# matteociccozzi/LayoutDiT

Hardware: AMD Instinct MI355X
Metric: images/sec ViT-B/16 224px bs=64 fwd (higher is better)
Workload: dtype f32; 1 GPU; ViT-base/16 224x224 bs=64 f32 forward, taps [4, 6, 8, 12] (BASELINE.json configs[1]); images_per_gpu=64, global_batch=64, parallelism=dp1: batch-sharded replicas, no data-path collective, weights=synthetic seed 0, images=synthetic doc-like pages, seed 1234, rank0_placement=128 CPUs: NUMA node 0 of GPU 0000:72:00.0

## Files before the change

include/ldit.h:

```cpp
#ifndef LDIT_H
#define LDIT_H

#include <stddef.h>
#include <stdint.h>

#ifdef __cplusplus
extern "C" {
#endif

#define LDIT_ABI_VERSION 6
#define LDIT_MAX_TAPS 8

enum ldit_status {
    LDIT_OK = 0,
    LDIT_EINVAL = -1,
    LDIT_EWORKSPACE = -2,
    LDIT_EHIP = -3,
    LDIT_EUNSUPPORTED = -4
};

enum ldit_dtype {
    LDIT_F32 = 0,
    LDIT_BF16 = 1,
    LDIT_FP8 = 3,
// ... 41 lines not shown
    const void *wq, *bq;
    const void *wk;
    const void *wv, *bv;
    const void *wo, *bo;
    const void *lam1;
    const void *ln2_w, *ln2_b;
    const void *w1, *b1;
    const void *w2, *b2;
    const void *lam2;
} ldit_layer_weights;

typedef struct ldit_weights {
    const void *patch_w;
    const void *patch_b;
    const void *cls;
    const void *pos;
    const ldit_layer_weights *layer;
} ldit_weights;

int ldit_abi_version(void);
const char *ldit_last_error(void);
int ldit_debug_reload_env(void);


size_t ldit_packed_bytes(const ldit_cfg *cfg);

int ldit_pack_weights(const ldit_cfg *cfg, const ldit_weights *w, void *packed, size_t packed_bytes, ldit_stream stream);

int ldit_set_fp8_act_scales(const ldit_cfg *cfg, void *packed, size_t packed_bytes, const float *act_scales,
                            ldit_stream stream);

size_t ldit_workspace_bytes(const ldit_cfg *cfg, int32_t batch);

int ldit_vit_forward(const ldit_cfg *cfg, const void *packed, const void *x, int32_t batch, void *const *tap_out,
                     void *workspace, size_t workspace_bytes, ldit_stream stream);

int ldit_vit_forward_images(const ldit_cfg *cfg, const void *packed, const void *const *images, const int32_t *heights,
                            const int32_t *widths, int32_t half_in, float mean, float std, int32_t batch, void *const *tap_out,
                            void *workspace, size_t workspace_bytes, ldit_stream stream);

enum ldit_kernel_family {
    LDIT_K_GEMM = 0,
    LDIT_K_ATTENTION = 1,
    LDIT_K_LAYERNORM = 2,
    LDIT_K_OTHER = 3,
    LDIT_K_COUNT = 4
};
int ldit_vit_forward_timed(const ldit_cfg *cfg, const void *packed, const void *x, int32_t batch, void *const *tap_out,
                           void *workspace, size_t workspace_bytes, ldit_stream stream, double *ms, int64_t *launches);


int ldit_linear_f32(const void *X, int64_t lda, const void *W, const void *bias, void *Y, int64_t ldy, int64_t M,
                    int64_t N, int64_t K, int32_t epilogue, const void *lam, const void *R, void *Y2,
                    ldit_stream stream);

int ldit_layernorm_f32(const void *X, const void *gamma, const void *beta, void *Y, int64_t rows, int64_t C, float eps,
                       ldit_stream stream);

int ldit_attention_f32(const void *Q, const void *K, const void *V, void *O, int64_t B, int64_t N, int64_t H,
                       int64_t D, int64_t ldq, int64_t ldk, int64_t ldv, int64_t ldo, float scale, ldit_stream stream);

int ldit_embed_f32(const void *x, const void *patch_w, const void *patch_b, const void *cls, const void *pos, void *out,
                   int64_t B, int64_t in_ch, int64_t img_h, int64_t img_w, int64_t p, int64_t C, ldit_stream stream);

int ldit_tap_to_map_f32(const void *tap, void *out, int64_t B, int64_t Gh, int64_t Gw, int64_t C, float scale,
                        ldit_stream stream);
// ... 200 lines not shown
```

layoutdit_amd/_lib.py:

```python
from __future__ import annotations

import ctypes as C
import os

_HERE = os.path.dirname(os.path.abspath(__file__))
LIB_PATH = os.environ.get("LDIT_LIB_PATH") or os.path.join(_HERE, "libldit_hip.so")

LDIT_ABI_VERSION = 6
LDIT_MAX_TAPS = 8
DTYPE_F32, DTYPE_BF16, DTYPE_FP8, DTYPE_F32X3, DTYPE_F32X6, DTYPE_MXFP8 = 0, 1, 3, 4, 5, 6
FP8_A_COUNT = 4
LDIT_OK, LDIT_EINVAL, LDIT_EWORKSPACE, LDIT_EHIP, LDIT_EUNSUPPORTED = 0, -1, -2, -3, -4
EPI_BIAS, EPI_BIAS_GELU, EPI_SCALE_RESID, EPI_F32, EPI_GELU_BWD = 0, 1, 2, 4, 5
K_GEMM, K_ATTENTION, K_LAYERNORM, K_OTHER, K_COUNT = 0, 1, 2, 3, 4
KERNEL_FAMILIES = ("gemm", "attention", "layernorm", "other")


class LditCfg(C.Structure):
    _fields_ = [("hidden", C.c_int32), ("layers", C.c_int32), ("heads", C.c_int32), ("mlp", C.c_int32),
                ("patch", C.c_int32), ("in_ch", C.c_int32), ("img_h", C.c_int32), ("img_w", C.c_int32),
                ("n_taps", C.c_int32), ("taps", C.c_int32 * LDIT_MAX_TAPS), ("ln_eps", C.c_float),
                ("dtype", C.c_int32), ("flags", C.c_int32)]


# ... 2 lines not shown


class LditLayerWeights(C.Structure):
    _fields_ = [(n, C.c_void_p) for n in LAYER_FIELDS]


class LditWeights(C.Structure):
    _fields_ = [("patch_w", C.c_void_p), ("patch_b", C.c_void_p), ("cls", C.c_void_p), ("pos", C.c_void_p),
                ("layer", C.POINTER(LditLayerWeights))]


class LditOptSegment(C.Structure):
    _fields_ = [("p", C.c_void_p), ("g", C.c_void_p), ("m", C.c_void_p), ("v", C.c_void_p), ("n", C.c_int64),
                ("bf16_mirror", C.c_void_p)]


class LditOptState(C.Structure):
    _fields_ = [("found_inf", C.c_int32), ("skip", C.c_int32), ("step", C.c_int32), ("growth_tracker", C.c_int32),
                ("skipped_steps", C.c_int32), ("scale", C.c_float), ("inv_scale_used", C.c_float), ("lr", C.c_float),
                ("bc1", C.c_float), ("bc2_sqrt", C.c_float)]


OPT_STATE_FIELDS = tuple(n for n, _ in LditOptState._fields_)
OPT_MAX_SEGMENTS = 64

_vp, _i64, _i32, _f32, _sz = C.c_void_p, C.c_int64, C.c_int32, C.c_float, C.c_size_t
SIGNATURES = {
    "ldit_abi_version": (C.c_int, []),
    "ldit_last_error": (C.c_char_p, []),
    "ldit_debug_reload_env": (C.c_int, []),
    "ldit_packed_bytes": (_sz, [C.POINTER(LditCfg)]),
    "ldit_pack_weights": (C.c_int, [C.POINTER(LditCfg), C.POINTER(LditWeights), _vp, _sz, _vp]),
    "ldit_workspace_bytes": (_sz, [C.POINTER(LditCfg), _i32]),
    "ldit_vit_forward": (C.c_int, [C.POINTER(LditCfg), _vp, _vp, _i32, C.POINTER(_vp), _vp, _sz, _vp]),
    "ldit_vit_forward_images": (C.c_int, [C.POINTER(LditCfg), _vp, C.POINTER(_vp), C.POINTER(_i32), C.POINTER(_i32), _i32, _f32, _f32, _i32,
                                          C.POINTER(_vp), _vp, _sz, _vp]),
    "ldit_vit_forward_timed": (C.c_int, [C.POINTER(LditCfg), _vp, _vp, _i32, C.POINTER(_vp), _vp, _sz, _vp,
                                         C.POINTER(C.c_double), C.POINTER(C.c_int64)]),
    "ldit_linear_f32": (C.c_int, [_vp, _i64, _vp, _vp, _vp, _i64, _i64, _i64, _i64, _i32, _vp, _vp, _vp, _vp]),
    "ldit_layernorm_f32": (C.c_int, [_vp, _vp, _vp, _vp, _i64, _i64, _f32, _vp]),
    "ldit_attention_f32": (C.c_int, [_vp, _vp, _vp, _vp, _i64, _i64, _i64, _i64, _i64, _i64, _i64, _i64, _f32, _vp]),
    "ldit_embed_f32": (C.c_int, [_vp, _vp, _vp, _vp, _vp, _vp, _i64, _i64, _i64, _i64, _i64, _i64, _vp]),
    "ldit_attention_planes": (C.c_int, [_vp, _vp, _vp, _vp, _i64, _i64, _i64, _i64, _i64, _i64, _i64, _i32, _vp]),
    "ldit_split_f32_planes": (C.c_int, [_vp, _i64, _vp, _i64, _i64, _i32, _vp]),
    "ldit_layernorm_f32_planes": (C.c_int, [_vp, _vp, _vp, _vp, _i64, _i64, C.c_float, _i32, _vp]),
    "ldit_linear_planes": (C.c_int, [_vp, _i64, _vp, _vp, _vp, _i64, _i64, _i64, _i64, _i32, _vp, _vp, _vp, _i32, _vp]),
    "ldit_embed_bf16": (C.c_int, [_vp, _vp, _vp, _vp, _vp, _vp, _vp, _i64, _i64, _i64, _i64, _i64, _i64, _vp]),
    "ldit_embed_bf16_images": (C.c_int, [C.POINTER(_vp), C.POINTER(_i32), C.POINTER(_i32), _i32, _f32, _f32, _vp, _vp, _vp, _vp, _vp, _vp,
                                         _i64, _i64, _i64, _i64, _i64, _i64, _vp]),
    "ldit_tap_to_map_f32": (C.c_int, [_vp, _vp, _i64, _i64, _i64, _i64, _f32, _vp]),
    "ldit_tap_to_map_bwd_f32": (C.c_int, [_vp, _vp, _i64, _i64, _i64, _i64, _f32, _vp]),
    "ldit_linear_bf16": (C.c_int, [_vp, _i64, _vp, _vp, _vp, _i64, _i64, _i64, _i64, _i32, _vp, _vp, _vp, _vp]),
    "ldit_attention_bf16": (C.c_int, [_vp, _vp, _vp, _vp, _i64, _i64, _i64, _i64, _i64, _i64, _i64, _i64, _f32, _vp]),
    "ldit_cast_f32_bf16": (C.c_int, [_vp, _vp, _i64, _vp]),
    "ldit_linear_fp8": (C.c_int, [_vp, _i64, _vp, _vp, _vp, _i64, _i64, _i64, _i64, _i32, _vp, _vp, _vp, _f32, _f32, _vp, _vp]),
    "ldit_quant_rows_f32_fp8": (C.c_int, [_vp, _vp, _vp, _i64, _i64, _vp]),
    "ldit_set_fp8_act_scales": (C.c_int, [C.POINTER(LditCfg), _vp, C.c_size_t, C.POINTER(C.c_float), _vp]),
    "ldit_quant_f32_fp8": (C.c_int, [_vp, _vp, _i64, _f32, _vp]),
    "ldit_quant_mx_f32_fp8": (C.c_int, [_vp, _i64, _vp, _vp, _i64, _i64, _vp]),
    "ldit_linear_mxfp8": (C.c_int, [_vp, _i64, _vp, _vp, _vp, _vp, _vp, _i64, _vp, _i64, _i64, _i64, _i32, _vp, _vp, _vp, _vp]),
    "ldit_layernorm_mxfp8": (C.c_int, [_vp, _vp, _vp, _vp, _vp, _i64, _i64, _f32, _vp]),
    "ldit_amax_f32": (C.c_int, [_vp, _i64, _vp, _vp]),
    "ldit_preprocess_f32": (C.c_int, [C.POINTER(_vp), C.POINTER(_i32), C.POINTER(_i32), _i32, _i32, _f32, _f32, _i32, _i32,
                                      _vp, _vp]),
    "ldit_preprocess_f16": (C.c_int, [C.POINTER(_vp), C.POINTER(_i32), C.POINTER(_i32), _i32, _i32, _f32, _f32, _i32, _i32,
                                      _vp, _vp]),
# ... 108 lines not shown
```

layoutdit_amd/csrc/api.hip:

```cpp
#include "api_internal.h"

namespace ldit {

char *err_buf()
{
    static thread_local char buf[512] = {0};
    return buf;
}

int fail(int code, const char *fmt, ...)
{
    va_list ap;
    va_start(ap, fmt);
    vsnprintf(err_buf(), 512, fmt, ap);
    va_end(ap);
    return code;
}

int ensure_dynamic_lds(const void *kern, int bytes, std::atomic<unsigned long long> &done)
{
    int dev = 0;
    LDIT_HIP_CHECK(hipGetDevice(&dev));
    const unsigned long long bit = dev >= 0 && dev < 64 ? 1ull << dev : 0ull;
    if (bit && (done.load(std::memory_order_relaxed) & bit)) return LDIT_OK;
    LDIT_HIP_CHECK(hipFuncSetAttribute(kern, hipFuncAttributeMaxDynamicSharedMemorySize, bytes));
    if (bit) done.fetch_or(bit, std::memory_order_relaxed);
    return LDIT_OK;
}

int compute_units()
{
    static std::atomic<int> cached[64];
    int dev = 0;
// ... 4 lines not shown
        if (c > 0) return c;
    }
    int n = 0;
    if (hipDeviceGetAttribute(&n, hipDeviceAttributeMultiprocessorCount, dev) != hipSuccess || n <= 0) n = 256;
    if (slot) cached[dev].store(n, std::memory_order_relaxed);
    return n;
}

namespace {
DiagSwitches read_switches()
{
    DiagSwitches d;
    auto digit = [](const char *name, int lo, int hi) {
        const char *e = getenv(name);
        return (e && e[0] >= '0' + lo && e[0] <= '0' + hi && e[1] == 0) ? e[0] - '0' : -1;
    };
    auto is = [](const char *name, char c) { const char *e = getenv(name); return e && e[0] == c; };
    d.gemm_tile = digit("LDIT_GEMM_TILE", 0, 7);
    if (const char *e = getenv("LDIT_GEMM_THIN_TILES")) d.thin_tiles = atol(e);
    d.panel_r16_vec = is("LDIT_PANEL_R16", 'v');
    d.panel_persist = is("LDIT_GEMM_PERSIST", '1');
    d.bf16_tile = digit("LDIT_GEMM_BF16_TILE", 2, 7);
    d.bf16_tile_env = getenv("LDIT_GEMM_BF16_TILE") != nullptr;
    d.bf16_tr_tile = digit("LDIT_GEMM_BF16_TR_TILE", 0, 9);
    d.bf16_tail_launch = is("LDIT_GEMM_BF16_TAIL_LAUNCH", '1');
    d.fp8_tile = digit("LDIT_GEMM_FP8_TILE", 0, 6);
    d.fp8_k16 = is("LDIT_GEMM_FP8_K16", '1');
    d.fp8_noskinny = is("LDIT_GEMM_FP8_NOSKINNY", '1');
    d.direct_epi = is("LDIT_GEMM_DIRECT_EPILOGUE", '1');
    d.attn_bf16_kt4 = is("LDIT_ATTN_BF16_KT", '4');
    d.seg_order = digit("LDIT_GEMM_SEG_ORDER", 0, 1);
    if (const char *e = getenv("LDIT_PLANES_TAIL_WAVES")) d.planes_tail_waves = atol(e);
    d.attn_bf16_nw = digit("LDIT_ATTN_BF16_NW", 4, 8);
    return d;
}
DiagSwitches &switches()
{
    static DiagSwitches d = read_switches();
    return d;
}
}

const DiagSwitches &diag() { return switches(); }
void reload_diag() { switches() = read_switches(); }

int embed(const Geo &g, const float *x, const float *pw, const float *pb, const float *cls, const float *pos, float *out,
          int batch, int img_h, int img_w, hipStream_t stream, Probe &probe)
{
    GemmArgs a{};
    a.A = x; a.W = pw; a.Y = out; a.Y2 = nullptr; a.bias = pb; a.pos = pos;
    a.M = batch * g.P; a.N = g.C; a.K = g.Kp;
    a.lda = g.in_ch * img_h * img_w;
    a.ldy = g.C;
    a.img_h = img_h; a.img_w = img_w; a.gw = g.gw; a.patches = g.P; a.patch = g.p; a.tokens = g.T;
    LDIT_RUN(probe, LDIT_K_GEMM, launch_gemm(a, EPI_EMBED, A_PATCH, stream));
    LDIT_RUN(probe, LDIT_K_OTHER, launch_cls_rows(cls, pos, out, batch, g.T, g.C, stream));
    return LDIT_OK;
}

int embed_bf16(const Geo &g, const float *x, const ImgSrc *imgs, int planes, void *patches, const void *w16, const float *pb,
               const float *cls, const float *pos, float *out, int batch, int img_h, int img_w, hipStream_t stream, Probe &probe)
{
    if (imgs)
        LDIT_RUN(probe, LDIT_K_OTHER, launch_patches_rows_images(imgs->images, imgs->half_in, imgs->heights, imgs->widths, batch, g.in_ch,
                                                                imgs->mean, imgs->std, img_h, img_w, g.p, patches, stream, planes));
    else
// ... 39 lines not shown
        }
        case LDIT_FP8:
            return launch_gemm_fp8(A.p, A.ld, W, bias, Y.p, Y.ld, M, N, K, epi, lam, R, Y2, ab_scale, out_inv_scale,
                                   static_cast<const float *>(A.s), static_cast<const float *>(Ws), static_cast<const float *>(Y.s), stream);
        case LDIT_MXFP8:
            if (b.train && epi != EPI_BIAS)
                return launch_gemm_mxfp8_train(A.p, A.ld, A.s, W, Ws, bias, Y.p, Y.ld, Y.s, M, N, K, epi, lam, R, Y2, t.Ypre, t.rowscale, t.Yd, stream);
            return launch_gemm_mxfp8(A.p, A.ld, A.s, W, Ws, bias, Y.p, Y.ld, Y.s, M, N, K, epi, lam, R, Y2, stream);
        default: return fail(LDIT_EUNSUPPORTED, "linear: no kernel for dtype %d", b.dtype);
    }
}

int attention(Build b, const void *Q, const void *K, const void *V, int ldq, int ldk, int ldv, const Operand &O, int B, int N, int H, int D,
              float scale, hipStream_t stream, float *lse, void *Ob, void *Od, int plane_in)
{
    switch (b.dtype) {
        case LDIT_F32:
            return launch_attention(static_cast<const float *>(Q), static_cast<const float *>(K), static_cast<const float *>(V),
                                    static_cast<float *>(O.p), B, N, H, D, ldq, ldk, ldv, O.ld, scale, stream);
        case LDIT_BF16:
            return b.train ? launch_attention_bf16_lse(Q, K, V, O.p, lse, B, N, H, D, ldq, ldk, ldv, O.ld, scale, stream)
                           : launch_attention_bf16(Q, K, V, O.p, B, N, H, D, ldq, ldk, ldv, O.ld, scale, stream);
        case LDIT_FP8:
            return launch_attention_bf16_fp8out(Q, K, V, O.p, B, N, H, D, ldq, ldk, ldv, O.ld, scale, static_cast<const float *>(O.s), stream);
        case LDIT_MXFP8:
            return b.train ? launch_attention_bf16_mxout_train(Q, K, V, O.p, O.s, lse, Ob, Od, B, N, H, D, ldq, ldk, ldv, O.ld, scale, stream)
                           : launch_attention_bf16_mxout(Q, K, V, O.p, O.s, B, N, H, D, ldq, ldk, ldv, O.ld, scale, stream);
        case LDIT_F32X3: case LDIT_F32X6:
            return (O.planes == 2 ? launch_attention_planes2 : launch_attention_planes3)(Q, K, V, O.p, B, N, H, D, ldq, plane_in, O.ld, stream);
        default: return fail(LDIT_EUNSUPPORTED, "attention: no kernel for dtype %d", b.dtype);
    }
}

int run_layer(Build b, const Geo &g, int batch, float eps, const Layer &d, hipStream_t stream, Probe &probe)
{
    const int M = batch * g.T, C = g.C, F = g.F;
    const char *q = static_cast<const char *>(d.qkv.p), *k = q + d.qk_bytes, *v = k + d.qk_bytes;
    const Operand mid = operand(d.h_mid, nullptr, C), out = operand(d.h_out, nullptr, C);
    const PackedLayer &pv = *d.v, &pw = *d.w;
    LDIT_RUN(probe, LDIT_K_LAYERNORM, layernorm(b, d.h_in, d.vec(pv.ln1_w), d.vec(pv.ln1_b), d.y1, d.y1d, M, C, eps, stream));
    LDIT_RUN(probe, LDIT_K_GEMM, linear(b, d.y1, d.mat(pw.wqkv), d.W + pw.sw_qkv, d.bqkv, d.qkv, M, 3 * C, C, EPI_BIAS, nullptr, nullptr, nullptr, Side{}, stream));
    LDIT_RUN(probe, LDIT_K_ATTENTION, attention(b, q, k, v, d.qkv.ld, d.qkv.ld, d.qkv.ld, d.o, batch, g.T, g.H, g.D, d.scale, stream, d.lse, d.ob, d.od,
                                                d.qkv.planes ? d.qkv.ld / d.qkv.planes : 0));
    LDIT_RUN(probe, LDIT_K_GEMM, linear(b, d.o, d.mat(pw.wo), d.W + pw.sw_o, d.vec(pv.bo), mid, M, C, C, EPI_SCALE_RESID, d.vec(pv.lam1), d.h_in, nullptr, d.s_o, stream));
    LDIT_RUN(probe, LDIT_K_LAYERNORM, layernorm(b, d.h_mid, d.vec(pv.ln2_w), d.vec(pv.ln2_b), d.y2, d.y2d, M, C, eps, stream));
    LDIT_RUN(probe, LDIT_K_GEMM, linear(b, d.y2, d.mat(pw.w1), d.W + pw.sw_1, d.vec(pv.b1), d.hid, M, F, C, EPI_BIAS_GELU, nullptr, nullptr, nullptr, d.s_fc1, stream));
    LDIT_RUN(probe, LDIT_K_GEMM, linear(b, d.hid, d.mat(pw.w2), d.W + pw.sw_2, d.vec(pv.b2), out, M, C, F, EPI_SCALE_RESID, d.vec(pv.lam2), d.h_mid, d.tap, d.s_fc2, stream));
    return LDIT_OK;
}

namespace {

Geo embed_geo(int64_t in_ch, int64_t img_h, int64_t img_w, int64_t p, int64_t C)
{
    Geo g{};
    g.C = (int)C; g.p = (int)p; g.in_ch = (int)in_ch; g.gh = (int)(img_h / p); g.gw = (int)(img_w / p);
    g.P = g.gh * g.gw; g.T = g.P + 1; g.Kp = (int)(in_ch * p * p);
    return g;
}

int embed_bf16_entry(const char *name, const void *x, const ImgSrc *imgs, const void *patch_w_bf16, const void *patch_b, const void *cls,
                     const void *pos, void *out, void *scratch, int64_t B, int64_t in_ch, int64_t img_h, int64_t img_w, int64_t p, int64_t C,
                     ldit_stream stream)
{
    if (B <= 0 || (imgs && B > 65535) || in_ch <= 0 || img_h <= 0 || img_w <= 0 || p <= 0 || C <= 0) return fail(LDIT_EINVAL, "%s: empty problem", name);
    if (img_h % p || img_w % p)
        return fail(LDIT_EINVAL, "%s: %s %lldx%lld is not a multiple of patch %lld", name, imgs ? "target" : "image", (long long)img_h, (long long)img_w, (long long)p);
    if ((imgs ? !imgs->images || !imgs->heights || !imgs->widths : !x) || !patch_w_bf16 || !patch_b || !cls || !pos || !out || !scratch)
        return fail(LDIT_EINVAL, "%s: null operand", name);
    if (imgs && !(imgs->std > 0.0f)) return fail(LDIT_EINVAL, "%s: std must be positive", name);
    if (!aligned16(out) || !aligned16(pos) || !aligned16(scratch) || !aligned16(patch_w_bf16) || (C & 3))
        return fail(LDIT_EINVAL, "%s: out / pos / scratch / patch_w must be 16-byte aligned, C a multiple of 4", name);
    const int64_t P = (img_h / p) * (img_w / p), Kp = in_ch * p * p;
    if (Kp % 64) return fail(LDIT_EUNSUPPORTED, "%s: in_ch*p*p = %lld must be a multiple of 64", name, (long long)Kp);
    if (B * in_ch * img_h * img_w >= (1ll << 31) || B * (P + 1) * C >= (1ll << 31) || B * P * Kp >= (1ll << 31))
        return fail(LDIT_EUNSUPPORTED, "%s: operand exceeds 2^31 elements", name);
    Probe probe;
    return embed_bf16(embed_geo(in_ch, img_h, img_w, p, C), static_cast<const float *>(x), imgs, 1, scratch, patch_w_bf16,
                      static_cast<const float *>(patch_b), static_cast<const float *>(cls), static_cast<const float *>(pos), static_cast<float *>(out),
                      (int)B, (int)img_h, (int)img_w, static_cast<hipStream_t>(stream), probe);
}

int linear_entry(const char *name, int dtype, const void *X, int64_t lda, const void *W, const void *bias, void *Y, int64_t ldy, int64_t M, int64_t N,
                 int64_t K, int32_t epilogue, const void *lam, const void *R, void *Y2, ldit_stream stream)
{
    LDIT_TRY(check_linear(name, M, N, K, lda, ldy, Y, Y2, epilogue));
    return linear(Build{dtype, false}, operand(X, nullptr, lda), W, nullptr, static_cast<const float *>(bias), operand(Y, nullptr, ldy), (int)M, (int)N,
                  (int)K, epilogue, static_cast<const float *>(lam), static_cast<const float *>(R), static_cast<float *>(Y2), Side{},
                  static_cast<hipStream_t>(stream));
}

int attention_entry(const char *name, int dtype, int64_t qtile, const void *Q, const void *K, const void *V, void *O, int64_t B, int64_t N, int64_t H,
                    int64_t D, int64_t ldq, int64_t ldk, int64_t ldv, int64_t ldo, float scale, ldit_stream stream)
{
    if (B <= 0 || N <= 0 || H <= 0) return fail(LDIT_EINVAL, "%s: empty problem", name);
    const int64_t ldmax = ldq > ldk ? (ldq > ldv ? ldq : ldv) : (ldk > ldv ? ldk : ldv);
    if (B * N * (ldmax > ldo ? ldmax : ldo) >= (1ll << 31) || B * H * ((N + qtile - 1) / qtile) >= (1ll << 31))
        return fail(LDIT_EUNSUPPORTED, "%s: operand exceeds 2^31 elements", name);
    if (ldq < H * D || ldk < H * D || ldv < H * D || ldo < H * D) return fail(LDIT_EINVAL, "%s: row stride smaller than H*D", name);
    return attention(Build{dtype, false}, Q, K, V, (int)ldq, (int)ldk, (int)ldv, operand(O, nullptr, ldo), (int)B, (int)N, (int)H, (int)D, scale,
                     static_cast<hipStream_t>(stream));
}

int preprocess(bool half_in, const void *const *images, const int32_t *heights, const int32_t *widths, int32_t B, int32_t in_ch, float mean,
               float std, int32_t out_h, int32_t out_w, void *out, ldit_stream stream)
{
    if (!images || !heights || !widths || !out) return fail(LDIT_EINVAL, "preprocess: null argument");
    if (B <= 0 || B > 65535 || in_ch <= 0 || out_h <= 0 || out_w <= 0) return fail(LDIT_EINVAL, "preprocess: bad geometry");
    if (!(std > 0.0f)) return fail(LDIT_EINVAL, "preprocess: std must be positive");
    if ((int64_t)B * in_ch * out_h * out_w >= (1ll << 31)) return fail(LDIT_EUNSUPPORTED, "preprocess: batch exceeds 2^31 elements");
    return launch_preprocess(images, half_in, heights, widths, B, in_ch, mean, std, out_h, out_w, static_cast<float *>(out),
                             static_cast<hipStream_t>(stream));
}

int forward(const ldit_cfg *cfg, const void *packed, const void *x, int32_t batch, void *const *tap_out, void *workspace,
            size_t ws_bytes, hipStream_t stream, Probe &probe, const ImgSrc *imgs = nullptr)
{
    Geo g;
    LDIT_TRY(geometry(cfg, g));
    LDIT_TRY(check_forward_args(cfg, g, batch, {packed, imgs ? packed : x, workspace}, "packed / x / workspace", imgs, tap_out));
    const int dt = cfg->dtype, S = split_planes_of(dt);
    const Workspace wm = workspace_map(g, batch, dt);
    if (ws_bytes < wm.total) return fail(LDIT_EWORKSPACE, "workspace %zu bytes < required %zu", ws_bytes, wm.total);
    const PackedMap pm = packed_map(g, dt);
    const char *P = static_cast<const char *>(packed);
    auto F32 = [&](size_t off) { return reinterpret_cast<const float *>(P + off); };
    char *ws = static_cast<char *>(workspace), *yb = ws + wm.y, *bb = ws + wm.big;
    float *h = reinterpret_cast<float *>(ws + wm.h);
    const int M = batch * g.T, C = g.C, F = g.F;
    const size_t act_bytes = (size_t)M * C * 4;

    if (dt != LDIT_F32 && g.Kp % 64 == 0) {
        LDIT_TRY(embed_bf16(g, static_cast<const float *>(x), imgs, S ? S : 1, bb, P + pm.patch_w16, F32(pm.patch_b), F32(pm.cls), F32(pm.pos), h,
                            batch, cfg->img_h, cfg->img_w, stream, probe));
    } else {
        const float *xp = static_cast<const float *>(x);
        if (imgs) {
            const size_t pix = (size_t)batch * g.in_ch * cfg->img_h * cfg->img_w * 4;
            if (wm.total - wm.big < pix) return fail(LDIT_EUNSUPPORTED, "image list: the pixel batch does not fit the workspace of this geometry");
            xp = reinterpret_cast<const float *>(bb);
            LDIT_RUN(probe, LDIT_K_OTHER, launch_preprocess(imgs->images, imgs->half_in, imgs->heights, imgs->widths, batch, g.in_ch, imgs->mean,
                                                           imgs->std, cfg->img_h, cfg->img_w, reinterpret_cast<float *>(bb), stream));
        }
        LDIT_TRY(embed(g, xp, F32(pm.patch_w), F32(pm.patch_b), F32(pm.cls), F32(pm.pos), h, batch, cfg->img_h, cfg->img_w, stream, probe));
    }
    LDIT_TRY(copy_taps(cfg, tap_out, 0, h, nullptr, act_bytes, stream));

    const bool mx = dt == LDIT_MXFP8;
    const int Sp = S ? S : 1;
    Layer d{};
    d.h_in = d.h_mid = d.h_out = h;
    d.V = d.W = P; d.div = 1;
    d.y1 = d.o = d.y2 = operand(yb, mx ? yb + (size_t)M * C : nullptr, Sp * C, S);
    d.qkv = operand(bb, nullptr, Sp * 3 * C, S);
    d.hid = operand(bb, mx ? bb + (size_t)M * F : nullptr, Sp * F, S);
    d.qk_bytes = (size_t)(dt == LDIT_F32 ? 4 : 2) * C;
    d.scale = dt == LDIT_F32 ? 1.0f / sqrtf((float)g.D) : 0.0f ;
    for (int l = 0; l < g.L; ++l) {
        const PackedLayer &pl = pm.layer[l];
        d.v = d.w = &pl; d.bqkv = F32(pl.bqkv);
        if (dt == LDIT_FP8) {
            const float *sc = F32(pl.scales);
            d.y1.s = const_cast<float *>(sc); d.o.s = const_cast<float *>(sc + 2); d.y2.s = const_cast<float *>(sc + 4); d.hid.s = const_cast<float *>(sc + 6);
        }
        d.tap = tap_of(cfg, tap_out, l + 1);
        LDIT_TRY(run_layer(Build{dt, false}, g, batch, cfg->ln_eps, d, stream, probe));
        if (d.tap) LDIT_TRY(copy_taps(cfg, tap_out, l + 1, h, d.tap, act_bytes, stream));
    }
    return LDIT_OK;
}

}
}

using namespace ldit;

extern "C" {

int ldit_abi_version(void) { return LDIT_ABI_VERSION; }

int ldit_debug_reload_env(void)
{
    reload_diag();
    return LDIT_OK;
}

const char *ldit_last_error(void) { return err_buf(); }

size_t ldit_packed_bytes(const ldit_cfg *cfg)
{
// ... 65 lines not shown
        LDIT_TRY(put(pl.bo, s.bo, C, "bo"));
        LDIT_TRY(put(pl.lam1, s.lam1, C, "lam1"));
        LDIT_TRY(put(pl.ln2_w, s.ln2_w, C, "ln2_w"));
        LDIT_TRY(put(pl.ln2_b, s.ln2_b, C, "ln2_b"));
        LDIT_TRY(put_mat(pl.w1, 0, s.w1, F, C, pl.sw_1, 0, "w1"));
        LDIT_TRY(put(pl.b1, s.b1, F, "b1"));
        LDIT_TRY(put_mat(pl.w2, 0, s.w2, C, F, pl.sw_2, 0, "w2"));
        LDIT_TRY(put(pl.b2, s.b2, C, "b2"));
        LDIT_TRY(put(pl.lam2, s.lam2, C, "lam2"));
    }
    return LDIT_OK;
}

int ldit_set_fp8_act_scales(const ldit_cfg *cfg, void *packed, size_t packed_bytes, const float *act_scales, ldit_stream stream_)
{
    Geo g;
    LDIT_TRY(geometry(cfg, g));
    if (cfg->dtype != LDIT_FP8) return fail(LDIT_EINVAL, "set_fp8_act_scales: cfg.dtype is not LDIT_FP8");
    if (!packed || !act_scales) return fail(LDIT_EINVAL, "set_fp8_act_scales: null pointer");
    const PackedMap pm = packed_map(g, cfg->dtype);
    if (packed_bytes < pm.total) return fail(LDIT_EWORKSPACE, "packed buffer %zu bytes < required %zu", packed_bytes, pm.total);
    hipStream_t stream = static_cast<hipStream_t>(stream_);
    char *P = static_cast<char *>(packed);
    for (int l = 0; l < g.L; ++l)
        for (int a = 0; a < LDIT_FP8_A_COUNT; ++a) {
            const float v = act_scales[l * LDIT_FP8_A_COUNT + a];
            if (!(v > 0.0f) || !std::isfinite(v)) return fail(LDIT_EINVAL, "set_fp8_act_scales: layer %d scale %d = %g is not positive", l, a, (double)v);
            LDIT_HIP_CHECK(hipMemcpyAsync(P + pm.layer[l].scales + 8 * a, &act_scales[l * LDIT_FP8_A_COUNT + a], sizeof(float),
                                          hipMemcpyHostToDevice, stream));
        }
    return LDIT_OK;
}

size_t ldit_workspace_bytes(const ldit_cfg *cfg, int32_t batch)
{
    Geo g;
    if (batch <= 0 || geometry(cfg, g) != LDIT_OK) return 0;
    return workspace_map(g, batch, cfg->dtype).total;
}

int ldit_vit_forward(const ldit_cfg *cfg, const void *packed, const void *x, int32_t batch, void *const *tap_out,
                     void *workspace, size_t workspace_bytes, ldit_stream stream)
{
    Probe probe;
    return forward(cfg, packed, x, batch, tap_out, workspace, workspace_bytes, static_cast<hipStream_t>(stream), probe);
}

int ldit_vit_forward_images(const ldit_cfg *cfg, const void *packed, const void *const *images, const int32_t *heights,
                            const int32_t *widths, int32_t half_in, float mean, float std, int32_t batch, void *const *tap_out,
                            void *workspace, size_t workspace_bytes, ldit_stream stream)
{
    Probe probe;
    const ImgSrc src{images, heights, widths, half_in != 0, mean, std};
    return forward(cfg, packed, nullptr, batch, tap_out, workspace, workspace_bytes, static_cast<hipStream_t>(stream), probe, &src);
}

int ldit_vit_forward_timed(const ldit_cfg *cfg, const void *packed, const void *x, int32_t batch, void *const *tap_out,
                           void *workspace, size_t workspace_bytes, ldit_stream stream, double *ms, int64_t *launches)
{
    if (!ms || !launches) return fail(LDIT_EINVAL, "ms / launches is null");
    Probe probe;
    probe.on = true;
    probe.stream = static_cast<hipStream_t>(stream);
    int rc = forward(cfg, packed, x, batch, tap_out, workspace, workspace_bytes, probe.stream, probe);
    int rc2 = probe.collect(ms, launches);
    return rc != LDIT_OK ? rc : rc2;
// ... 276 lines not shown
```

layoutdit_amd/csrc/api_internal.h:

```cpp
#pragma once
#include <algorithm>
#include <initializer_list>
#include <cmath>
#include <cstring>
#include <vector>

#include "ldit_common.h"

namespace ldit {

inline size_t up(size_t v, size_t a) { return (v + a - 1) / a * a; }

struct Geo {
    int C, L, H, F, D, p, in_ch, gh, gw, P, T, Kp;
};

inline int split_planes_of(int dtype) { return dtype == LDIT_F32X3 ? 2 : dtype == LDIT_F32X6 ? 3 : 0; }

inline int geometry(const ldit_cfg *cfg, Geo &g)
{
    if (!cfg) return fail(LDIT_EINVAL, "cfg is null");
    if (cfg->dtype != LDIT_F32 && cfg->dtype != LDIT_BF16 && cfg->dtype != LDIT_FP8 && cfg->dtype != LDIT_MXFP8 && !split_planes_of(cfg->dtype))
        return fail(LDIT_EUNSUPPORTED, "dtype %d: only fp32 (0), bf16 (1), fp8 e4m3 (3), split fp32 (4, 5) and MX fp8 (6) are implemented",
                    cfg->dtype);
// ... 133 lines not shown

#define LDIT_RUN(probe, family, expr)  \
    do {                               \
        LDIT_TRY((probe).begin(family)); \
        LDIT_TRY(expr);                \
        LDIT_TRY((probe).end());       \
    } while (0)

inline float qfold_of(const Geo &g) { return (1.0f / sqrtf((float)g.D)) * 1.44269504088896340736f; }

inline GemmExtra split_segments(int planes)
{
    GemmExtra x{};
    if (planes == 2) { x.nseg = 3; x.seg_a = 0x001u; x.seg_w = 0x010u; }
    if (planes == 3) { x.nseg = 6; x.seg_a = 0x001012u; x.seg_w = 0x010210u; }
    x.seg_inner = x.nseg != 0;
    return x;
}

struct ImgSrc {
    const void *const *images;
    const int32_t *heights, *widths;
    bool half_in;
    float mean, std;
};

inline float *tap_of(const ldit_cfg *cfg, void *const *taps, int hidden_idx)
{
    for (int i = 0; taps && i < cfg->n_taps; ++i)
        if (cfg->taps[i] == hidden_idx && taps[i]) return static_cast<float *>(taps[i]);
    return nullptr;
}

inline int copy_taps(const ldit_cfg *cfg, void *const *taps, int hidden_idx, const float *src, const float *already, size_t bytes, hipStream_t stream)
{
    for (int i = 0; i < cfg->n_taps; ++i)
        if (cfg->taps[i] == hidden_idx && taps[i] != already)
            LDIT_HIP_CHECK(hipMemcpyAsync(taps[i], src, bytes, hipMemcpyDeviceToDevice, stream));
    return LDIT_OK;
}

inline int check_forward_args(const ldit_cfg *cfg, const Geo &g, int batch, std::initializer_list<const void *> ptrs, const char *names,
                              const ImgSrc *imgs, void *const *tap_out)
{
    if (batch <= 0) return fail(LDIT_EINVAL, "batch %d must be positive", batch);
    for (const void *p : ptrs)
        if (!p) return fail(LDIT_EINVAL, "null %s pointer", names);
    for (const void *p : ptrs)
        if (!aligned16(p)) return fail(LDIT_EINVAL, "pointers must be 16-byte aligned");
    if (imgs && (!imgs->images || !imgs->heights || !imgs->widths || !(imgs->std > 0.0f) || batch > 65535))
        return fail(LDIT_EINVAL, "image list: null array, non-positive std or more than 65535 images");
    if (cfg->n_taps && !tap_out) return fail(LDIT_EINVAL, "tap_out is null");
    for (int i = 0; i < cfg->n_taps; ++i)
        if (!tap_out[i] || !aligned16(tap_out[i])) return fail(LDIT_EINVAL, "tap_out[%d] is null or misaligned", i);
    if ((int64_t)batch * g.T * (int64_t)(g.F > 3 * g.C ? g.F : 3 * g.C) >= (1ll << 31))
        return fail(LDIT_EUNSUPPORTED, "batch %d: activation index space exceeds 2^31 elements, split the batch", batch);
    return LDIT_OK;
}

inline int check_linear(const char *name, int64_t M, int64_t N, int64_t K, int64_t lda, int64_t ldy, const void *Y, const void *Y2,
                        int epilogue = LDIT_EPI_BIAS, int64_t planes = 1)
{
    if (M <= 0 || N <= 0 || K <= 0) return fail(LDIT_EINVAL, "%s: empty problem", name);
    if (M * (ldy > lda ? ldy : lda) >= (1ll << 31) || N * K * planes >= (1ll << 31)) return fail(LDIT_EUNSUPPORTED, "%s: operand exceeds 2^31 elements", name);
    if ((planes == 1 && ldy < N) || lda < planes * K) return fail(LDIT_EINVAL, "%s: bad leading dimension", name);
    if (!Y || !aligned16(Y) || (Y2 && !aligned16(Y2))) return fail(LDIT_EINVAL, "%s: output null or misaligned", name);
    if (epilogue < LDIT_EPI_BIAS || epilogue > LDIT_EPI_SCALE_RESID) return fail(LDIT_EINVAL, "%s: unknown epilogue %d", name, epilogue);
    return LDIT_OK;
}

struct Build { int dtype; bool train; };

struct Operand {
    void *p = nullptr;
    void *s = nullptr;
    int ld = 0;
    int planes = 0;
};
inline Operand operand(const void *p, const void *s, int64_t ld, int planes = 0) { return {const_cast<void *>(p), const_cast<void *>(s), (int)ld, planes}; }

struct Side { void *Ypre = nullptr; const float *rowscale = nullptr; void *Yd = nullptr; };

struct Layer {
    const float *h_in; float *h_mid, *h_out;
    Operand y1, qkv, o, y2, hid;
    size_t qk_bytes;
    float scale;
    const char *V, *W; const PackedLayer *v, *w; size_t div; const float *bqkv;
    const float *vec(size_t off) const { return reinterpret_cast<const float *>(V + off); }
    const void *mat(size_t off) const { return W + off / div; }
    float *tap;
    Side s_o, s_fc1, s_fc2;
    float *lse; void *y1d, *y2d, *ob, *od;
};

int layernorm(Build b, const float *X, const float *gamma, const float *beta, const Operand &Y, void *Yd, int64_t rows, int C, float eps, hipStream_t stream);
int linear(Build b, const Operand &A, const void *W, const void *Ws, const float *bias, const Operand &Y, int M, int N, int K, int epi, const float *lam,
           const float *R, float *Y2, const Side &t, hipStream_t stream, float ab_scale = 0.f, float out_inv_scale = 0.f);
int attention(Build b, const void *Q, const void *K, const void *V, int ldq, int ldk, int ldv, const Operand &O, int B, int N, int H, int D, float scale,
              hipStream_t stream, float *lse = nullptr, void *Ob = nullptr, void *Od = nullptr, int plane_in = 0);
int run_layer(Build b, const Geo &g, int batch, float eps, const Layer &d, hipStream_t stream, Probe &probe);
int embed(const Geo &g, const float *x, const float *pw, const float *pb, const float *cls, const float *pos, float *out, int batch, int img_h, int img_w, hipStream_t stream, Probe &probe);
int embed_bf16(const Geo &g, const float *x, const ImgSrc *imgs, int planes, void *patches, const void *w16, const float *pb, const float *cls,
               const float *pos, float *out, int batch, int img_h, int img_w, hipStream_t stream, Probe &probe);

}
```

layoutdit_amd/csrc/ldit_common.h:

```cpp
#pragma once
#include <hip/hip_runtime.h>

#include <atomic>
#include <cstdarg>
#include <cstdint>
#include <cstdio>

#include "ldit.h"

namespace ldit {

typedef float f32x2 __attribute__((ext_vector_type(2)));
typedef float f32x4 __attribute__((ext_vector_type(4)));
typedef float f32x16 __attribute__((ext_vector_type(16)));

char *err_buf();
int fail(int code, const char *fmt, ...);

#define LDIT_HIP_CHECK(expr)                                                                              \
    do {                                                                                                  \
        hipError_t e__ = (expr);                                                                          \
        if (e__ != hipSuccess) return ::ldit::fail(LDIT_EHIP, "%s: %s", #expr, hipGetErrorString(e__));   \
    } while (0)

static inline bool aligned16(const void *p) { return (reinterpret_cast<uintptr_t>(p) & 15u) == 0; }

int ensure_dynamic_lds(const void *kern, int bytes, std::atomic<unsigned long long> &done);
#define LDIT_DYN_LDS(kern, bytes)                                                                               \
    do {                                                                                                        \
        static std::atomic<unsigned long long> done__{0};                                                       \
        if (int rc__ = ::ldit::ensure_dynamic_lds(reinterpret_cast<const void *>(kern), (bytes), done__)) return rc__; \
    } while (0)

int compute_units();

struct DiagSwitches {
    int gemm_tile = -1;
    long thin_tiles = 192;
    bool panel_r16_vec = false;
    bool panel_persist = false;
    int bf16_tile = -1;
    bool bf16_tile_env = false;
    int bf16_tr_tile = -1;
    bool bf16_tail_launch = false;
    int fp8_tile = -1;
    bool fp8_k16 = false, fp8_noskinny = false;
    bool direct_epi = false;
    bool attn_bf16_kt4 = false;
    int attn_bf16_nw = -1;
    long planes_tail_waves = 700;
    int seg_order = -1;
};
const DiagSwitches &diag();
void reload_diag();

__device__ __forceinline__ float erf_fast(float a)
{
    const float t = fabsf(a), s = a * a;
    float r = fmaf(-1.72853470e-5f, t, 3.83197126e-4f);
    const float u = fmaf(-3.88396438e-3f, t, 2.42546219e-2f);
    r = fmaf(r, s, u);
    r = fmaf(r, t, -1.06777877e-1f);
    r = fmaf(r, t, -6.34846687e-1f);
    r = fmaf(r, t, -1.28717512e-1f);
    r = fmaf(r, t, -t);
    const float big = copysignf(1.0f - __expf(r), a);
    float q = -5.96761703e-4f;
    q = fmaf(q, s, 4.99119423e-3f);
    q = fmaf(q, s, -2.67681349e-2f);
    q = fmaf(q, s, 1.12819925e-1f);
    q = fmaf(q, s, -3.76125336e-1f);
    q = fmaf(q, s, 1.28379166e-1f);
    const float small = fmaf(q, a, a);
    return t > 0.927734375f ? big : small;
}

__device__ __forceinline__ float gelu_erf(float v) { return 0.5f * v * (1.0f + erf_fast(v * 0.70710678118654752440f)); }

__device__ __forceinline__ float gelu_lp(float v)
{
    const float w = v * __builtin_fmaf(v * v, -0.10294324f, -2.30220819f);
    return v * __builtin_amdgcn_rcpf(1.0f + __builtin_amdgcn_exp2f(w));
}

// ... 223 lines not shown
```

Baseline: 3435 images/sec.

## Split f32 forward batch into two lanes on concurrent streams

For f32 with at least 48 images, the batch is split in half and each half's transformer layers are enqueued on its own stream, the main one and a persistent non-blocking side stream, interleaved launch by launch. Fork and join events tie the side stream back to the caller's stream. The aim is to overlap the two halves' kernels so each gap between launches and any under-filled kernel is covered by the other half. The risk is that each GEMM gets half the rows, which lowers per-kernel efficiency, and the two lanes compete for CUs and cache. The lane split is skipped during graph capture and when profiling probes are on.

```diff
diff --git a/include/ldit.h b/include/ldit.h
--- a/include/ldit.h
+++ b/include/ldit.h
@@ -97,6 +97,8 @@
 
 size_t ldit_workspace_bytes(const ldit_cfg *cfg, int32_t batch);
 
+int32_t ldit_forward_lanes(const ldit_cfg *cfg, int32_t batch);
+
 int ldit_vit_forward(const ldit_cfg *cfg, const void *packed, const void *x, int32_t batch, void *const *tap_out,
                      void *workspace, size_t workspace_bytes, ldit_stream stream);
 
diff --git a/layoutdit_amd/_lib.py b/layoutdit_amd/_lib.py
--- a/layoutdit_amd/_lib.py
+++ b/layoutdit_amd/_lib.py
@@ -58,6 +58,7 @@
     "ldit_packed_bytes": (_sz, [C.POINTER(LditCfg)]),
     "ldit_pack_weights": (C.c_int, [C.POINTER(LditCfg), C.POINTER(LditWeights), _vp, _sz, _vp]),
     "ldit_workspace_bytes": (_sz, [C.POINTER(LditCfg), _i32]),
+    "ldit_forward_lanes": (_i32, [C.POINTER(LditCfg), _i32]),
     "ldit_vit_forward": (C.c_int, [C.POINTER(LditCfg), _vp, _vp, _i32, C.POINTER(_vp), _vp, _sz, _vp]),
     "ldit_vit_forward_images": (C.c_int, [C.POINTER(LditCfg), _vp, C.POINTER(_vp), C.POINTER(_i32), C.POINTER(_i32), _i32, _f32, _f32, _i32,
                                           C.POINTER(_vp), _vp, _sz, _vp]),
diff --git a/layoutdit_amd/csrc/api.hip b/layoutdit_amd/csrc/api.hip
--- a/layoutdit_amd/csrc/api.hip
+++ b/layoutdit_amd/csrc/api.hip
@@ -1,4 +1,6 @@
 #include "api_internal.h"
+
+#include <mutex>
 
 namespace ldit {
 
@@ -69,6 +71,7 @@
     d.seg_order = digit("LDIT_GEMM_SEG_ORDER", 0, 1);
     if (const char *e = getenv("LDIT_PLANES_TAIL_WAVES")) d.planes_tail_waves = atol(e);
     d.attn_bf16_nw = digit("LDIT_ATTN_BF16_NW", 4, 8);
+    d.fwd_lanes = digit("LDIT_FWD_LANES", 1, 2);
     return d;
 }
 DiagSwitches &switches()
@@ -174,21 +177,52 @@
     }
 }
 
-int run_layer(Build b, const Geo &g, int batch, float eps, const Layer &d, hipStream_t stream, Probe &probe)
+int layer_launch(int i, Build b, const Geo &g, int batch, float eps, const Layer &d, hipStream_t stream, Probe &probe)
 {
     const int M = batch * g.T, C = g.C, F = g.F;
     const char *q = static_cast<const char *>(d.qkv.p), *k = q + d.qk_bytes, *v = k + d.qk_bytes;
     const Operand mid = operand(d.h_mid, nullptr, C), out = operand(d.h_out, nullptr, C);
     const PackedLayer &pv = *d.v, &pw = *d.w;
-    LDIT_RUN(probe, LDIT_K_LAYERNORM, layernorm(b, d.h_in, d.vec(pv.ln1_w), d.vec(pv.ln1_b), d.y1, d.y1d, M, C, eps, stream));
-    LDIT_RUN(probe, LDIT_K_GEMM, linear(b, d.y1, d.mat(pw.wqkv), d.W + pw.sw_qkv, d.bqkv, d.qkv, M, 3 * C, C, EPI_BIAS, nullptr, nullptr, nullptr, Side{}, stream));
-    LDIT_RUN(probe, LDIT_K_ATTENTION, attention(b, q, k, v, d.qkv.ld, d.qkv.ld, d.qkv.ld, d.o, batch, g.T, g.H, g.D, d.scale, stream, d.lse, d.ob, d.od,
-                                                d.qkv.planes ? d.qkv.ld / d.qkv.planes : 0));
-    LDIT_RUN(probe, LDIT_K_GEMM, linear(b, d.o, d.mat(pw.wo), d.W + pw.sw_o, d.vec(pv.bo), mid, M, C, C, EPI_SCALE_RESID, d.vec(pv.lam1), d.h_in, nullptr, d.s_o, stream));
-    LDIT_RUN(probe, LDIT_K_LAYERNORM, layernorm(b, d.h_mid, d.vec(pv.ln2_w), d.vec(pv.ln2_b), d.y2, d.y2d, M, C, eps, stream));
-    LDIT_RUN(probe, LDIT_K_GEMM, linear(b, d.y2, d.mat(pw.w1), d.W + pw.sw_1, d.vec(pv.b1), d.hid, M, F, C, EPI_BIAS_GELU, nullptr, nullptr, nullptr, d.s_fc1, stream));
-    LDIT_RUN(probe, LDIT_K_GEMM, linear(b, d.hid, d.mat(pw.w2), d.W + pw.sw_2, d.vec(pv.b2), out, M, C, F, EPI_SCALE_RESID, d.vec(pv.lam2), d.h_mid, d.tap, d.s_fc2, stream));
-    return LDIT_OK;
+    switch (i) {
+        case 0:
+            LDIT_RUN(probe, LDIT_K_LAYERNORM, layernorm(b, d.h_in, d.vec(pv.ln1_w), d.vec(pv.ln1_b), d.y1, d.y1d, M, C, eps, stream));
+            return LDIT_OK;
+        case 1:
+            LDIT_RUN(probe, LDIT_K_GEMM, linear(b, d.y1, d.mat(pw.wqkv), d.W + pw.sw_qkv, d.bqkv, d.qkv, M, 3 * C, C, EPI_BIAS, nullptr, nullptr, nullptr, Side{}, stream));
+            return LDIT_OK;
+        case 2:
+            LDIT_RUN(probe, LDIT_K_ATTENTION, attention(b, q, k, v, d.qkv.ld, d.qkv.ld, d.qkv.ld, d.o, batch, g.T, g.H, g.D, d.scale, stream, d.lse, d.ob, d.od,
+                                                        d.qkv.planes ? d.qkv.ld / d.qkv.planes : 0));
+            return LDIT_OK;
+        case 3:
+            LDIT_RUN(probe, LDIT_K_GEMM, linear(b, d.o, d.mat(pw.wo), d.W + pw.sw_o, d.vec(pv.bo), mid, M, C, C, EPI_SCALE_RESID, d.vec(pv.lam1), d.h_in, nullptr, d.s_o, stream));
+            return LDIT_OK;
+        case 4:
+            LDIT_RUN(probe, LDIT_K_LAYERNORM, layernorm(b, d.h_mid, d.vec(pv.ln2_w), d.vec(pv.ln2_b), d.y2, d.y2d, M, C, eps, stream));
+            return LDIT_OK;
+        case 5:
+            LDIT_RUN(probe, LDIT_K_GEMM, linear(b, d.y2, d.mat(pw.w1), d.W + pw.sw_1, d.vec(pv.b1), d.hid, M, F, C, EPI_BIAS_GELU, nullptr, nullptr, nullptr, d.s_fc1, stream));
+            return LDIT_OK;
+        case 6:
+            LDIT_RUN(probe, LDIT_K_GEMM, linear(b, d.hid, d.mat(pw.w2), d.W + pw.sw_2, d.vec(pv.b2), out, M, C, F, EPI_SCALE_RESID, d.vec(pv.lam2), d.h_mid, d.tap, d.s_fc2, stream));
+            return LDIT_OK;
+        default: return fail(LDIT_EINVAL, "layer_launch: no launch %d", i);
+    }
+}
+
+int run_layer(Build b, const Geo &g, int batch, float eps, const Layer &d, hipStream_t stream, Probe &probe)
+{
+    for (int i = 0; i < LAYER_LAUNCHES; ++i) LDIT_TRY(layer_launch(i, b, g, batch, eps, d, stream, probe));
+    return LDIT_OK;
+}
+
+constexpr int FWD_LANES_MIN_ROWS = 48 * 197;
+
+int forward_lanes(int dtype, const Geo &g, int batch)
+{
+    if (dtype != LDIT_F32 || batch < 2) return 1;
+    if (const int force = diag().fwd_lanes; force > 0) return force;
+    return (int64_t)batch * g.T >= FWD_LANES_MIN_ROWS ? 2 : 1;
 }
 
 namespace {
@@ -255,6 +289,53 @@
                              static_cast<hipStream_t>(stream));
 }
 
+int side_stream(hipStream_t &out)
+{
+    static std::mutex mu;
+    static hipStream_t streams[64] = {};
+    int dev = 0;
+    LDIT_HIP_CHECK(hipGetDevice(&dev));
+    out = nullptr;
+    if (dev < 0 || dev >= 64) return LDIT_OK;
+    std::lock_guard<std::mutex> lock(mu);
+    if (!streams[dev]) LDIT_HIP_CHECK(hipStreamCreateWithFlags(&streams[dev], hipStreamNonBlocking));
+    out = streams[dev];
+    return LDIT_OK;
+}
+
+int enqueue_lanes(const ldit_cfg *cfg, const Geo &g, const PackedMap &pm, const Layer &full, char *yb, char *bb, int batch, void *const *tap_out,
+                  hipStream_t stream, hipStream_t side, hipEvent_t start, bool &forked, Probe &probe)
+{
+    const int C = g.C, F = g.F, bA = (batch + 1) / 2;
+    const size_t wide = (size_t)(3 * C > F ? 3 * C : F);
+    const char *P = full.V;
+    struct Lane { Layer d; int batch; size_t row0; hipStream_t s; } lane[2] = {{full, bA, 0, stream}, {full, batch - bA, (size_t)bA * g.T, side}};
+    for (Lane &n : lane) {
+        float *h = const_cast<float *>(full.h_in) + n.row0 * C;
+        n.d.h_in = n.d.h_mid = n.d.h_out = h;
+        n.d.y1 = n.d.o = n.d.y2 = operand(yb + n.row0 * C * 4, nullptr, C);
+        n.d.qkv = operand(bb + n.row0 * wide * 4, nullptr, 3 * C);
+        n.d.hid = operand(bb + n.row0 * wide * 4, nullptr, F);
+    }
+    LDIT_HIP_CHECK(hipEventRecord(start, stream));
+    LDIT_HIP_CHECK(hipStreamWaitEvent(side, start, 0));
+    forked = true;
+    for (int at = 0; at < g.L * LAYER_LAUNCHES; ++at)
+        for (Lane &n : lane) {
+            const int l = at / LAYER_LAUNCHES, i = at % LAYER_LAUNCHES;
+            if (i == 0) {
+                const PackedLayer &pl = pm.layer[l];
+                n.d.v = n.d.w = &pl; n.d.bqkv = reinterpret_cast<const float *>(P + pl.bqkv);
+                float *tap = tap_of(cfg, tap_out, l + 1);
+                n.d.tap = tap ? tap + n.row0 * C : nullptr;
+            }
+            LDIT_TRY(layer_launch(i, Build{LDIT_F32, false}, g, n.batch, cfg->ln_eps, n.d, n.s, probe));
+            if (i == LAYER_LAUNCHES - 1 && n.d.tap)
+                LDIT_TRY(copy_taps(cfg, tap_out, l + 1, full.h_in, tap_of(cfg, tap_out, l + 1), (size_t)n.batch * g.T * C * 4, n.s, n.row0 * C * 4));
+        }
+    return LDIT_OK;
+}
+
 int forward(const ldit_cfg *cfg, const void *packed, const void *x, int32_t batch, void *const *tap_out, void *workspace,
             size_t ws_bytes, hipStream_t stream, Probe &probe, const ImgSrc *imgs = nullptr)
 {
@@ -298,6 +379,32 @@
     d.hid = operand(bb, mx ? bb + (size_t)M * F : nullptr, Sp * F, S);
     d.qk_bytes = (size_t)(dt == LDIT_F32 ? 4 : 2) * C;
     d.scale = dt == LDIT_F32 ? 1.0f / sqrtf((float)g.D) : 0.0f ;
+
+    hipStream_t side = nullptr;
+    if (!probe.on && g.L > 0 && forward_lanes(dt, g, batch) == 2) {
+        hipStreamCaptureStatus cap = hipStreamCaptureStatusNone;
+        LDIT_HIP_CHECK(hipStreamIsCapturing(stream, &cap));
+        if (cap == hipStreamCaptureStatusNone) LDIT_TRY(side_stream(side));
+    }
+    if (side) {
+        if (C & 3) return fail(LDIT_EINVAL, "forward: hidden %d is not a multiple of 4, lane rows would lose their 16-byte alignment", C);
+        hipEvent_t start = nullptr, done = nullptr;
+        LDIT_HIP_CHECK(hipEventCreateWithFlags(&start, hipEventDisableTiming));
+        if (hipError_t e = hipEventCreateWithFlags(&done, hipEventDisableTiming); e != hipSuccess) {
+            (void)hipEventDestroy(start);
+            return fail(LDIT_EHIP, "hipEventCreateWithFlags: %s", hipGetErrorString(e));
+        }
+        bool forked = false;
+        int rc = enqueue_lanes(cfg, g, pm, d, yb, bb, batch, tap_out, stream, side, start, forked, probe);
+        if (forked) {
+            hipError_t e = hipEventRecord(done, side);
+            if (e == hipSuccess) e = hipStreamWaitEvent(stream, done, 0);
+            if (e != hipSuccess && rc == LDIT_OK) rc = fail(LDIT_EHIP, "forward: joining the side stream: %s", hipGetErrorString(e));
+        }
+        (void)hipEventDestroy(start);
+        (void)hipEventDestroy(done);
+        return rc;
+    }
     for (int l = 0; l < g.L; ++l) {
         const PackedLayer &pl = pm.layer[l];
         d.v = d.w = &pl; d.bqkv = F32(pl.bqkv);
@@ -429,6 +536,13 @@
     return LDIT_OK;
 }
 
+int32_t ldit_forward_lanes(const ldit_cfg *cfg, int32_t batch)
+{
+    Geo g;
+    if (batch <= 0 || geometry(cfg, g) != LDIT_OK) return 0;
+    return forward_lanes(cfg->dtype, g, batch);
+}
+
 size_t ldit_workspace_bytes(const ldit_cfg *cfg, int32_t batch)
 {
     Geo g;
diff --git a/layoutdit_amd/csrc/api_internal.h b/layoutdit_amd/csrc/api_internal.h
--- a/layoutdit_amd/csrc/api_internal.h
+++ b/layoutdit_amd/csrc/api_internal.h
@@ -189,11 +189,13 @@
     return nullptr;
 }
 
-inline int copy_taps(const ldit_cfg *cfg, void *const *taps, int hidden_idx, const float *src, const float *already, size_t bytes, hipStream_t stream)
+inline int copy_taps(const ldit_cfg *cfg, void *const *taps, int hidden_idx, const float *src, const float *already, size_t bytes, hipStream_t stream,
+                     size_t offset = 0)
 {
     for (int i = 0; i < cfg->n_taps; ++i)
         if (cfg->taps[i] == hidden_idx && taps[i] != already)
-            LDIT_HIP_CHECK(hipMemcpyAsync(taps[i], src, bytes, hipMemcpyDeviceToDevice, stream));
+            LDIT_HIP_CHECK(hipMemcpyAsync(static_cast<char *>(taps[i]) + offset, reinterpret_cast<const char *>(src) + offset, bytes,
+                                          hipMemcpyDeviceToDevice, stream));
     return LDIT_OK;
 }
 
@@ -257,6 +259,9 @@
 int attention(Build b, const void *Q, const void *K, const void *V, int ldq, int ldk, int ldv, const Operand &O, int B, int N, int H, int D, float scale,
               hipStream_t stream, float *lse = nullptr, void *Ob = nullptr, void *Od = nullptr, int plane_in = 0);
 int run_layer(Build b, const Geo &g, int batch, float eps, const Layer &d, hipStream_t stream, Probe &probe);
+constexpr int LAYER_LAUNCHES = 7;
+int layer_launch(int i, Build b, const Geo &g, int batch, float eps, const Layer &d, hipStream_t stream, Probe &probe);
+int forward_lanes(int dtype, const Geo &g, int batch);
 int embed(const Geo &g, const float *x, const float *pw, const float *pb, const float *cls, const float *pos, float *out, int batch, int img_h, int img_w, hipStream_t stream, Probe &probe);
 int embed_bf16(const Geo &g, const float *x, const ImgSrc *imgs, int planes, void *patches, const void *w16, const float *pb, const float *cls,
                const float *pos, float *out, int batch, int img_h, int img_w, hipStream_t stream, Probe &probe);
diff --git a/layoutdit_amd/csrc/ldit_common.h b/layoutdit_amd/csrc/ldit_common.h
--- a/layoutdit_amd/csrc/ldit_common.h
+++ b/layoutdit_amd/csrc/ldit_common.h
@@ -50,6 +50,7 @@
     int attn_bf16_nw = -1;
     long planes_tail_waves = 700;
     int seg_order = -1;
+    int fwd_lanes = -1;
 };
 const DiagSwitches &diag();
 void reload_diag();
```

Result: faster. 3505 images/sec, median of 6 (+2.0%).
